# JanWosnitza/FrayTracer

Measured on AMD Instinct MI355X. Metric: Mrays/s (primary+secondary) at 4096x4096; max per-pixel |delta| vs F# ref (delta is measured against the CPU oracle: F# parity is unpinned, DESIGN.md section 2), higher is better.
Workload: dtype f32

## Files before the change

### fraytracer_amd/csrc/ft_kernels.h

```cpp
#pragma once
#include <hip/hip_runtime_api.h>
#include <stddef.h>
#include <stdint.h>

#include "../../include/fraytracer_hip.h"
#include "ft_device.h"
#include "ft_libm.h"

#define FT_BLOCK 256
#define FT_LDS_CNT_WORDS 64
#define FT_LDS_TILE_WORD 40
static_assert(FT_LDS_TILE_WORD >= 36 && FT_LDS_TILE_WORD + 2 * (256 / 64) <= FT_LDS_CNT_WORDS, "the tile words lie behind the clocks, inside the header");
#ifdef FT_UNION_PROFILE
#define FT_LDS_DBG_ROWS 13
#else
#define FT_LDS_DBG_ROWS 0
#endif
#define FT_SH_ROWS 10
#define FT_LDS_SH_BASE (FT_LDS_CNT_WORDS + FT_LDS_DBG_ROWS * FT_BLOCK)
#define FT_LDS_HDR_FLOATS (FT_LDS_SH_BASE + FT_SH_ROWS * FT_BLOCK)
#define FT_CULL_MAX 256
#define FT_CULL_ROW (4 * FT_CULL_MAX)

struct FtLdsLayout { uint32_t slotD, slotL, consts, libmTab, rows, total; };
FT_HD FtLdsLayout ft_lds_layout(uint32_t nSlots, uint32_t nStage, bool libm, bool rows) {
    FtLdsLayout L;
    L.slotD = FT_LDS_HDR_FLOATS;
    L.slotL = FT_LDS_HDR_FLOATS + nSlots * FT_BLOCK;
    L.consts = FT_LDS_HDR_FLOATS + 2u * nSlots * FT_BLOCK;
    L.libmTab = (L.consts + nStage + 1u) & ~1u;
    const uint32_t end = libm ? L.libmTab + 2u * FT_LIBM_TAB_DOUBLES : L.consts + nStage;
    L.rows = (end + 3u) & ~3u;
    L.total = rows ? L.rows + FT_CULL_ROW * (FT_BLOCK / 64) : end;
    return L;
// ... 122 lines not shown
```

### fraytracer_amd/csrc/kernels.hip

```cpp
#include <hip/hip_runtime.h>

#include "../../include/fraytracer_hip.h"
#include "ft_device.h"
#include "ft_kernels.h"
#include "ft_math.h"
#include "ft_libm.h"

#define FT_CONST __attribute__((address_space(4)))
typedef const float FT_CONST* cfp;
template <class T> __device__ __forceinline__ const T FT_CONST* as_const(const T* p) {
    return (const T FT_CONST*)(p);
}

__device__ __forceinline__ f3 ld3(cfp c) { return mk3(c[0], c[1], c[2]); }
__device__ __forceinline__ FtInstr ld_instr(const FtInstr FT_CONST* q) {
    FtInstr r; r.op = q->op; r.dst = q->dst; r.src = q->src; r.type = q->type; r.count = q->count; r.data = q->data;
    r.aux = q->aux; r.flags = q->flags; r.f0 = q->f0; r.f1 = q->f1; r.pad0 = 0; r.pad1 = 0; return r;
}
typedef float v4f __attribute__((ext_vector_type(4)));
typedef uint32_t v4u __attribute__((ext_vector_type(4)));
struct ItemRegs { v4f a; v4u b; };
__device__ __forceinline__ ItemRegs ld_item(const FtItemRec FT_CONST* q) {
    ItemRegs r;
    r.a = *reinterpret_cast<const v4f FT_CONST*>(q);
// ... 345 lines not shown
        uint32_t typeData, mat;
        if (first || (mn > lbA && mn > mdA)) { typeData = ra.b.y; mat = ra.b.z; i += 1u; }
        else {
            if (!(mn > lbA)) break;
            if (j == i || !(mn > lbB)) break;
            i += 2u;
            if (!(mn > mdB)) continue;
            typeData = rb.b.y; mat = rb.b.z;
        }
        FT_UDBG(2, 1); FT_UDBG_WAVE(3);
        FT_UDBG_T0(tPrim);
        float d; uint32_t l;
        ft_candidate<FQ, false>(typeData, mat, consts, p, sd, sl, d, l, [](uint32_t, float&, uint32_t&) {});
        FT_UDBG_T1(9, tPrim);
        if (first) { mn = d; leaf = l; first = false; if (mn <= cap && mn < capBound) break; }
        else {
            if (d < mn) leaf = l;
            mn = ft_min(mn, d);
        }
    }
    FT_UDBG_T1(4, tWalk);
    outD = mn; outLeaf = leaf;
}

#define FT_CULL_NONE 0xffffffffu
#define FT_CULL_NOCLAMP 0x10000u
template <bool WITH_UNION, bool CALLS, int MATH, bool COOP = false>
__device__ __forceinline__ void ft_exec(const FtSceneDev& S, uint32_t pc, uint32_t pcEnd, const f3 p, float* __restrict__ sd,
                                        uint32_t* __restrict__ sl, const float* __restrict__ ldsC, bool fastOk, bool nearOk, float epsHit = __builtin_inff(),
                                        const float* __restrict__ cullRow = nullptr, uint32_t cullN = FT_CULL_NONE);

template <bool FQ, int MATH>
__device__ __forceinline__ void eval_union(const FtSceneDev& S, const FtGrid FT_CONST& g, const f3 p,
                                           float* __restrict__ sd, uint32_t* __restrict__ sl, const float* __restrict__ ldsC,
                                           bool fastOk, bool nearOk, float& outD, uint32_t& outLeaf, float cap, float capBound) {
    const uint32_t cell = g.cellBase + ft_grid_cell(g, p);
    cfp ctr = as_const(S.cellCenters) + 3u * cell;
    const float distanceToCenter = ft_distance(mk3(ctr[0], ctr[1], ctr[2]), p);
    const uint32_t FT_CONST* cellStart = as_const(S.cellStart);
    const FtItemRec FT_CONST* items = as_const(S.items);
    cfp consts = as_const(S.consts);
    uint32_t i = cellStart[cell];
    const uint32_t end = cellStart[cell + 1];

    float mn = 0.0f; uint32_t leaf = 0;
    bool first = true;
// ... 199 lines not shown
__device__ __forceinline__ f3 ft_readlane3(f3 v, int l) {
    return mk3(__int_as_float(__builtin_amdgcn_readlane(__float_as_int(v.x), l)), __int_as_float(__builtin_amdgcn_readlane(__float_as_int(v.y), l)),
               __int_as_float(__builtin_amdgcn_readlane(__float_as_int(v.z), l)));
}
template <int CTRL> __device__ __forceinline__ float ft_dpp(float old, float v) {
    return __int_as_float(__builtin_amdgcn_update_dpp(__float_as_int(old), __float_as_int(v), CTRL, 0xf, 0xf, false));
}
__device__ __forceinline__ float ft_readlane_f(float v, int l) { return __int_as_float(__builtin_amdgcn_readlane(__float_as_int(v), l)); }
__device__ __forceinline__ float ft_wave_max_all(float v) {
    v = __builtin_fmaxf(v, ft_dpp<0x111>(0.0f, v)); v = __builtin_fmaxf(v, ft_dpp<0x112>(0.0f, v));
    v = __builtin_fmaxf(v, ft_dpp<0x114>(0.0f, v)); v = __builtin_fmaxf(v, ft_dpp<0x118>(0.0f, v));
    return __builtin_fmaxf(__builtin_fmaxf(ft_readlane_f(v, 15), ft_readlane_f(v, 31)), __builtin_fmaxf(ft_readlane_f(v, 47), ft_readlane_f(v, 63)));
}
__device__ __forceinline__ float ft_wave_scan_incl(float v, float& total) {
    const uint32_t lane = threadIdx.x & 63u;
    v += ft_dpp<0x111>(0.0f, v); v += ft_dpp<0x112>(0.0f, v); v += ft_dpp<0x114>(0.0f, v); v += ft_dpp<0x118>(0.0f, v);
    const float r0 = ft_readlane_f(v, 15), r1 = ft_readlane_f(v, 31), r2 = ft_readlane_f(v, 47), r3 = ft_readlane_f(v, 63);
    const float p2 = r0 + r1, p3 = p2 + r2;
    v += lane >= 48u ? p3 : (lane >= 32u ? p2 : (lane >= 16u ? r0 : 0.0f));
    total = p3 + r3;
    return v;
}
__device__ __forceinline__ float ft_wave_shift_right1(float v) { return ft_dpp<0x138>(0.0f, v); }
__device__ __forceinline__ uint32_t ft_cull_children(const FtSceneDev& S, const f3 p, bool active, unsigned long long am,
                                                     const float* __restrict__ ldsC, float* __restrict__ row) {
    if (S.cullPc == FT_CULL_NONE) return FT_CULL_NONE;
    const FtInstr FT_CONST* in = as_const(S.instr) + S.cullPc;
    const uint32_t flags = in->flags, count = in->count;
    const float si = in->f0;
    if (in->op != FT_OP_SMOOTH_RUN || !(flags & FT_FLAG_FAST) || count < FT_CULL_MIN || !(si < 0.0f)) return FT_CULL_NONE;
    if (!fast_point_ok(p, active)) return FT_CULL_NONE;
    const uint32_t lane = threadIdx.x & 63u;
    const f3 q00 = ft_readlane3(p, __ffsll((long long)am) - 1);
    const float fx = p.x - q00.x, fy = p.y - q00.y, fz = p.z - q00.z;
    const float far2 = active ? (fx * fx + fy * fy) + fz * fz : 0.0f;
    const float farMax = ft_wave_max_all(far2);
    const unsigned long long fm = __ballot(active && far2 == farMax);
    const f3 q01 = ft_readlane3(p, __ffsll((long long)(fm != 0ull ? fm : am)) - 1);
    const f3 q0 = mk3(0.5f * (q00.x + q01.x), 0.5f * (q00.y + q01.y), 0.5f * (q00.z + q01.z));
    const float ex = p.x - q0.x, ey = p.y - q0.y, ez = p.z - q0.z;
    const float rho2 = ft_wave_max_all(active ? (ex * ex + ey * ey) + ez * ez : 0.0f);
    const float rho = __builtin_amdgcn_sqrtf(rho2) * 1.001f + 1e-6f;
    const uint32_t n = count < FT_CULL_MAX ? count : FT_CULL_MAX;
    const float4* src = reinterpret_cast<const float4*>(ldsC + in->data);
    float4* dst = reinterpret_cast<float4*>(row);
    float carry = 0.0f;
    uint32_t kept = 0;
    bool apart = true;
    for (uint32_t base = 0; base < n; base += 64u) {
// ... 270 lines not shown
    {-0x1.21c850p-1f, 0x1.1e0d66p-3f, -0x1.a00000p-1f}, {0x1.38c4f8p-2f, 0x1.55799ap-3f, -0x1.e00000p-1f}};

struct LaneState {
    uint32_t phase, job, steps, lidx, leaf, outIdx;
    uint32_t certAt;
    f3 o, dir;
    float len, eps;
    uint32_t xs;
    f3 thr;
    uint32_t seed;
    __device__ __forceinline__ uint32_t aoIdx() const { return xs & 255u; }
    __device__ __forceinline__ uint32_t aoOpen() const { return (xs >> 8) & 255u; }
    __device__ __forceinline__ uint32_t bounce() const { return (xs >> 16) & 255u; }
    __device__ __forceinline__ bool inside() const { return (xs >> 31) != 0u; }
};

__device__ __forceinline__ void write_rgb(float* __restrict__ out, uint32_t idx, f3 c) {
    float* o = out + 3ull * idx;
    o[0] = c.x; o[1] = c.y; o[2] = c.z;
}

__device__ __forceinline__ f3 ft_background(const FtRenderArgs& a) { return mk3(a.S.bg[0], a.S.bg[1], a.S.bg[2]); }

template <bool EXT>
__device__ __forceinline__ void emit(const FtRenderArgs& a, const LaneState& s, f3 c) {
    write_rgb(a.out, s.outIdx, EXT ? c * s.thr : c);
}

__device__ __forceinline__ uint32_t ft_glass_hash(uint32_t seed, uint32_t bounce) {
    uint32_t h = seed + (bounce + 1u) * 0x27D4EB2Fu;
    h ^= h >> 16; h *= 0x7FEB352Du; h ^= h >> 15; h *= 0x846CA68Bu; h ^= h >> 16;
    return h;
}

__device__ __forceinline__ void write_try_trace_miss(const FtRenderArgs& a, const LaneState& s) {
    float* o = a.out + 10ull * s.outIdx;
    for (uint32_t i = 0; i < 10u; ++i) o[i] = 0.0f;
}
__device__ __forceinline__ void write_ray(float* o, f3 origin, f3 dir, float len, float eps) {
    o[0] = origin.x; o[1] = origin.y; o[2] = origin.z; o[3] = dir.x; o[4] = dir.y; o[5] = dir.z; o[6] = len; o[7] = eps;
}

template <bool VIEWS = false>
__device__ __forceinline__ bool ends_hit_segment(const FtRenderArgs& a, const LaneState& s) {
    if (VIEWS) return a.hits != 0u && (s.job / a.jobsPerPlane) % a.spp == 0u && s.bounce() == 0u;
    return a.hits != 0u && s.job < a.jobsPerPlane && s.bounce() == 0u;
// ... 221 lines not shown
        holds = holds || (t <= a.occ.reach && nSteps < 131072.0f && hitM <= a.occ.cap && (dist + hitM) * 1.001f < D);
    }
    return ok && holds;
}

__device__ __forceinline__ int first_step_from_cache(LaneState& s) {
    if (s.len <= 0.0f) return 0;
    const float d = *ft_sh(FT_SH_D0);
    if (d != d) { ft_flag(1u); return 2; }
    if (d < s.eps) return 1;
    s.o = s.o + s.dir * d;
    s.len = s.len - d;
    s.steps = 1;
    return 0;
}

struct FtLit { f3 lint, ldir; };
__device__ __forceinline__ FtLit ft_light_at(const uint32_t type, const f3 lv, const f3 lc, const f3 hp) {
    f3 lint = lc, ldir = lv;
    if (type != FT_LIGHT_DIRECTIONAL) { ldir = ft_normalize(lv - hp); lint = lint / ft_length2(lv - hp); }
    return FtLit{lint, ldir};
}

template <bool EXT, int FORM = FT_FORM_FRAME>
__device__ __forceinline__ void settle(const FtRenderArgs& a, LaneState& s) {
    constexpr bool VIEWS = FORM == FT_FORM_VIEWS, SHADE = FORM == FT_FORM_SHADE || FORM == FT_FORM_VIS, VIS = FORM == FT_FORM_VIS;
    const float piInv = 1.0f / 3.14159274101257324f;
    for (;;) {
        if (!SHADE && s.phase == PH_MARCH) {
            if (s.len <= 0.0f || ((!EXT || !s.inside()) && ft_never_enters(a.S, s.o, s.dir, s.eps, s.len))) {
                if (EXT && a.mode == 2u) write_try_trace_miss(a, s);
                else {
                    if (EXT && ends_hit_segment<VIEWS>(a, s)) write_hit_miss(a, hit_index<VIEWS>(a, s));
                    if (!EXT || a.hits != 2u) emit<EXT>(a, s, ft_background(a));
                }
                s.phase = PH_IDLE;
            }
            return;
        }
        if (EXT && s.phase == PH_AO) {
            if (s.len <= 0.0f) { s.xs += 0x101u; s.phase = PH_AONEXT; continue; }
            return;
        }
        if (EXT && s.phase == PH_AONEXT) {
            if (s.aoIdx() >= a.aoSamples) {
                const float f = (float)s.aoOpen() / (float)a.aoSamples;
                sh_set3(FT_SH_LACC, ft_background(a) * f);
                s.lidx = 0; s.phase = PH_LIGHTS;
                continue;
            }
            const f3 dir = ft_normalize(sh_get3(FT_SH_NRM) + mk3(FT_AO_DIRS[s.aoIdx()][0], FT_AO_DIRS[s.aoIdx()][1], FT_AO_DIRS[s.aoIdx()][2]));
            ft_count(FT_C_EXT);
            if (dir.x != dir.x || dir.y != dir.y || dir.z != dir.z) { s.xs += 0x101u; continue; }
            s.o = sh_get3(FT_SH_HP); s.dir = dir; s.len = a.aoRadius; s.steps = 0;
            s.phase = PH_AO;
            if (a.reuse != 0u) {
                const int r = first_step_from_cache(s);
                if (r == 1) { s.xs += 1u; s.phase = PH_AONEXT; }
                else if (r == 2) s.len = -1.0f;
            }
            continue;
        }
        if (s.phase == PH_SHADOW) {
            if (s.len <= 0.0f || ((!EXT || !s.inside()) && ft_never_enters(a.S, s.o, s.dir, s.eps, s.len))) {
                if (VIS) {
                    *ft_vis_word() |= 1u << s.lidx;
                    s.lidx += 1; s.phase = PH_LIGHTS;
                    continue;
                }
                const FtLight L = ld_light(as_const(a.S.lights) + s.lidx);
                const f3 lv = mk3(L.v[0], L.v[1], L.v[2]), hp = sh_get3(FT_SH_HP);
                const FtLit li = ft_light_at(L.type, lv, mk3(L.color[0], L.color[1], L.color[2]), hp);
                sh_set3(FT_SH_LACC, sh_get3(FT_SH_LACC) + li.lint * ft_dot(sh_get3(FT_SH_NRM), li.ldir));
                s.lidx += 1; s.phase = PH_LIGHTS;
                continue;
            }
            return;
        }
        if (s.phase == PH_LIGHTS) {
            if (VIS && s.lidx >= a.S.nLights) {
                a.visOut[s.job] = *ft_vis_word();
                s.phase = PH_IDLE;
                return;
            }
            if (VIS && ((a.visSel >> s.lidx) & 1u) == 0u) { s.lidx += 1; continue; }
            if (!VIS && s.lidx >= a.S.nLights) {
                cfp m = SHADE ? as_const(a.hitsIn) + 16ull * s.job + 11u : as_const(a.S.materials) + 3u * s.leaf;
                const f3 color = mk3(m[0], m[1], m[2]);
                emit<EXT>(a, s, color * (sh_get3(FT_SH_LACC) * piInv));
                s.phase = PH_IDLE;
                return;
            }
            const FtLight L = ld_light(as_const(a.S.lights) + s.lidx);
            const f3 lv = mk3(L.v[0], L.v[1], L.v[2]);
            const f3 hp = sh_get3(FT_SH_HP);
            const f3 ldir = ft_light_at(L.type, lv, mk3(L.color[0], L.color[1], L.color[2]), hp).ldir;
            const float lightCos = ft_dot(sh_get3(FT_SH_NRM), ldir);
            if (lightCos > 0.0f) {
                s.o = hp;
                if (L.type == FT_LIGHT_DIRECTIONAL) {
                    s.dir = lv; s.len = 1000.0f;
                } else {
                    const f3 diff = lv - hp;
                    const float distance2 = ft_length2(diff);
                    s.dir = diff / distance2;
                    s.len = sqrtf(distance2);
                }
                s.steps = 0; ft_count(FT_C_SHADOW);
                s.phase = PH_SHADOW; s.certAt = a.certShadow;
                if (!SHADE && a.reuse != 0u) {
                    const int r = first_step_from_cache(s);
                    if (r == 1) { ft_count(FT_C_HITS); s.lidx += 1; s.phase = PH_LIGHTS; }
                    else if (r == 2) s.len = -1.0f;
                }
                continue;
            }
            s.lidx += 1;
            continue;
        }
        return;
    }
}

struct ViewCam { f3 o, fw, up, rt; float d; uint32_t leaf; };

template <bool EXT, int FORM = FT_FORM_FRAME>
__device__ __forceinline__ void start_job(const FtRenderArgs& a, LaneState& s, const bool camKnown, float dCam, uint32_t leafCam, const ViewCam& vc) {
    constexpr bool VIEWS = FORM == FT_FORM_VIEWS, SHADE = FORM == FT_FORM_SHADE || FORM == FT_FORM_VIS, VIS = FORM == FT_FORM_VIS;
    if (SHADE) {
        const v4f FT_CONST* r = reinterpret_cast<const v4f FT_CONST*>(as_const(a.hitsIn) + 16ull * s.job);
        const v4f r0 = r[0], r1 = r[1], r2 = r[2], r3 = r[3];
        s.outIdx = s.job;
        s.eps = r1.w;
        s.steps = 0;
        const uint32_t kept = VIS ? (a.visIn ? a.visIn[s.job] & a.visKeep : 0u) : 0u;
        if (VIS && __float_as_uint(r3.z) == 0u) {
            a.visOut[s.job] = kept;
            s.phase = PH_IDLE;
            return;
        }
        if (__float_as_uint(r3.z) == 0u) {
            write_rgb(a.out, s.outIdx, ft_background(a));
            s.phase = PH_IDLE;
            return;
        }
        sh_set3(FT_SH_HP, mk3(r0.x, r0.y, r0.z));
        sh_set3(FT_SH_NRM, mk3(r2.x, r2.y, r2.z));
        if (VIS) *ft_vis_word() = kept;
        else sh_set3(FT_SH_LACC, ft_background(a));
        s.lidx = 0;
        s.phase = PH_LIGHTS;
        settle<EXT, FORM>(a, s);
        return;
    }
    if (a.mode >= 1) {
        const ft_ray r = a.rays[s.job];
        s.o = mk3(r.origin.x, r.origin.y, r.origin.z);
        s.dir = mk3(r.direction.x, r.direction.y, r.direction.z);
        s.len = r.length; s.eps = r.epsilon;
        s.outIdx = s.job;
        if (EXT) { s.thr = splat3(1.0f); s.seed = s.job; }
    } else {
        const uint32_t plane = (EXT || VIEWS) ? s.job / a.jobsPerPlane : 0u;
        const uint32_t smp = VIEWS ? (EXT ? plane % a.spp : 0u) : plane, jp = s.job - plane * a.jobsPerPlane;
        const uint32_t t = jp >> 6, i = jp & 63u;
        const uint32_t tx = t / a.tilesY, ty = t - tx * a.tilesY;
        const uint32_t cl = tx * 8u + (i >> 3), y = ty * 8u + (i & 7u);
        if (cl >= (uint32_t)a.nCols || y >= (uint32_t)a.H) { s.phase = PH_IDLE; return; }
        const uint32_t x = (uint32_t)a.x0 + (cl / a.stripeW) * (a.stripeW * a.stripeRanks) + a.stripeRank * a.stripeW + cl % a.stripeW;
        const float ox = EXT ? (float)(smp % a.sppN) / (float)a.sppN : 0.0f, oy = EXT ? (float)(smp / a.sppN) / (float)a.sppN : 0.0f;
        const float px = EXT ? ((float)x + ox) / a.maxSize : (float)x / a.maxSize;
        const float py = EXT ? ((float)y + oy) / a.maxSize : (float)y / a.maxSize;
        const f3 fw = VIEWS ? vc.fw : mk3(a.cam[3], a.cam[4], a.cam[5]), up = VIEWS ? vc.up : mk3(a.cam[6], a.cam[7], a.cam[8]);
        const f3 rt = VIEWS ? vc.rt : mk3(a.cam[9], a.cam[10], a.cam[11]);
        s.o = VIEWS ? vc.o : mk3(a.cam[0], a.cam[1], a.cam[2]);
        s.dir = ft_normalize(fw + (px - 0.5f) * rt + (py - 0.5f) * up);
        s.len = a.length; s.eps = a.eps;
        s.outIdx = plane * a.planePixels + cl * (uint32_t)a.H + y;
        if (VIEWS) { dCam = vc.d; leafCam = vc.leaf; }
        if (EXT) {
            s.thr = splat3(1.0f);
            if (a.spectral != 0u) { const uint32_t bin = smp % a.spectral; s.thr = mk3(a.spec[bin][0], a.spec[bin][1], a.spec[bin][2]); }
            s.seed = x * 0x9E3779B1u + y * 0x85EBCA77u + smp * 0xC2B2AE3Du;
        }
    }
    if (EXT) s.xs &= 0xffffu;
    s.steps = 0; ft_count(FT_C_PRIMARY);
    s.phase = PH_MARCH; s.certAt = a.certPrim;
    if (camKnown && s.len > 0.0f) {
        if (dCam != dCam) { ft_flag(1u); s.len = -1.0f; }
        else if (dCam < s.eps) { ft_count(FT_C_HITP); s.leaf = leafCam; s.phase = PH_NX; }
        else { s.o = s.o + s.dir * dCam; s.len = s.len - dCam; s.steps = 1; }
    }
    settle<EXT, FORM>(a, s);
}

__device__ __forceinline__ void glass_bounce(const FtRenderArgs& a, LaneState& s) {
    cfp mx = as_const(a.materialsExt) + 4u * s.leaf;
    const bool glass = mx[0] != 0.0f;
    const f3 black = mk3(0.0f, 0.0f, 0.0f);
    if (!glass) {
        if (s.inside()) { write_rgb(a.out, s.outIdx, black); s.phase = PH_IDLE; }
        return;
    }
    const f3 N = sh_get3(FT_SH_NRM), D = s.dir, hp = sh_get3(FT_SH_HP);
    if (s.bounce() >= a.maxBounces || N.x != N.x || N.y != N.y || N.z != N.z) { write_rgb(a.out, s.outIdx, black); s.phase = PH_IDLE; return; }
    float cosi = -ft_dot(N, D);
    if (!(cosi > 0.0f)) cosi = 0.0f;
    float n = mx[1];
    if (a.spectral != 0u) {
        const uint32_t smp = s.job / a.jobsPerPlane;
        n = mx[1] + mx[2] * a.spec[smp % a.spectral][3];
    }
    const float n1 = !s.inside() ? 1.0f : n, n2 = !s.inside() ? n : 1.0f;
    const float eta = n1 / n2;
    const float k = 1.0f - (eta * eta) * (1.0f - cosi * cosi);
    bool reflect = true;
// ... 2 lines not shown
        cost = sqrtf(k);
        float rs, rp;
        { const float p = n2 * cosi, q = n1 * cost, x = (p - q) / (p + q); rs = x * x; }
        { const float p = n1 * cosi, q = n2 * cost, x = (p - q) / (p + q); rp = x * x; }
        const float reflectance = 0.5f * (rs + rp);
        const float u = (float)(ft_glass_hash(s.seed, s.bounce()) >> 8) * (1.0f / 16777216.0f);
        reflect = u < reflectance;
    }
    ft_count(FT_C_EXT);
    if (reflect) {
        s.dir = ft_normalize(D + N * (2.0f * cosi));
        s.o = hp + N * (2.0f * s.eps);
    } else {
        s.dir = ft_normalize(D * eta + N * (eta * cosi - cost));
        s.o = hp - N * (4.0f * s.eps);
        s.xs ^= 0x80000000u;
        if (s.inside()) { cfp t = as_const(a.S.materials) + 3u * s.leaf; s.thr = s.thr * mk3(t[0], t[1], t[2]); }
    }
    s.xs += 0x10000u;
    s.len = a.length; s.steps = 0;
    s.phase = PH_MARCH; s.certAt = a.certPrim;
}

__device__ __forceinline__ unsigned long long wave_sum(uint32_t v) {
    unsigned long long x = v;
    for (int off = 32; off > 0; off >>= 1) x += __shfl_down(x, off, 64);
    return x;
}

template <int VARIANT, bool EXT, int MATH = 0, int K = 0, int FORM = FT_FORM_FRAME>
__device__ __forceinline__ void ft_trace_body(const FtRenderArgs& a) {
    constexpr bool VIEWS = FORM == FT_FORM_VIEWS, SHADE = FORM == FT_FORM_SHADE || FORM == FT_FORM_VIS;
    static_assert(!SHADE || !EXT, "ft_shade_hits and ft_light_visibility have no EXTENSION build");
    const uint32_t tid = threadIdx.x, lane = tid & 63u;
    unsigned long long* clk0 = reinterpret_cast<unsigned long long*>(ft_lds + 32);
    if (blockIdx.x == 0 && tid == 0) { clk0[0] = clock64(); clk0[1] = wall_clock64(); }
    const FtLdsLayout L = ft_lds_layout(a.S.nSlots, a.S.nStage, MATH != 0, true);
    float* sd = ft_lds + L.slotD + tid;
    uint32_t* sl = reinterpret_cast<uint32_t*>(ft_lds + L.slotL) + tid;
    float* ldsC = ft_lds + L.consts;
    for (uint32_t i = tid; i < a.S.nStage; i += FT_BLOCK) ldsC[i] = a.S.consts[i];
    if (MATH != 0 && tid < FT_LIBM_TAB_DOUBLES) const_cast<ft_u64*>(ft_libm_tab(a.S))[tid] = ft_libm_tab_g[tid];
    if (tid < 32u) reinterpret_cast<uint32_t*>(ft_lds)[tid] = 0u;
#ifdef FT_UNION_PROFILE
    for (uint32_t k = 0; k < FT_LDS_DBG_ROWS; ++k) reinterpret_cast<uint32_t*>(ft_lds)[FT_LDS_CNT_WORDS + tid + k * FT_BLOCK] = 0u;
#endif
    __syncthreads();

    float* coopRow = ft_lds + ft_lds_layout(a.S.nSlots, a.S.nStage, MATH != 0, true).rows + (uint32_t)__builtin_amdgcn_readfirstlane((int)(tid >> 6)) * FT_CULL_ROW;
    uint32_t cullSkipped = 0, cullTotal = 0;
    uint32_t chunkNext = 0, chunkEnd = 0;
    uint32_t waveEvals = 0;
    constexpr bool ORDER = FORM == FT_FORM_FRAME && !EXT && VARIANT == 1;
    uint32_t* tileSt = reinterpret_cast<uint32_t*>(ft_lds) + FT_LDS_TILE_WORD + (tid >> 6);
    constexpr uint32_t TILE_EVALS = FT_BLOCK / 64;
    if (ORDER && lane == 0) tileSt[0] = 0xffffffffu;
    uint32_t coopEvals = 0;
    uint32_t nEvals = 0;
    bool exhausted = false;
    LaneState s;
    s.phase = PH_IDLE; s.job = 0; s.steps = 0; s.lidx = 0; s.leaf = 0; s.outIdx = 0; s.certAt = 0xffffffffu;
    s.o = s.dir = mk3(0, 0, 0);
    s.len = 0; s.eps = 0;
    s.xs = 0;
    s.thr = splat3(1.0f); s.seed = 0;
    bool camKnown = false;
    float dCam = 0.0f; uint32_t leafCam = 0u;
    if (!SHADE && a.reuse != 0u && a.mode == 0u) {
        s.phase = PH_CAM;
        if (VIEWS) { const float* c = a.views + 12u * (lane % a.nViews); s.o = mk3(c[0], c[1], c[2]); }
        else s.o = mk3(a.cam[0], a.cam[1], a.cam[2]);
        s.eps = a.eps;
    }
    ViewCam vc{};

    for (;;) {
        for (int round = 0; round < 3; ++round) {
            const unsigned long long idle = __ballot(s.phase == PH_IDLE);
            if (idle == 0ull) break;
            if ((uint32_t)__popcll(idle) < a.refillMin && __ballot(s.phase >= PH_MARCH) != 0ull) break;
            if (chunkNext == chunkEnd) {
                if (exhausted) break;
                if (ORDER && a.tileCost != nullptr && lane == 0) {
                    const uint32_t t = tileSt[0];
                    if (t < (a.nJobs >> 6)) a.tileCost[t] = waveEvals - tileSt[TILE_EVALS];
                    tileSt[0] = 0xffffffffu;
                }
                uint32_t base = 0, take = a.chunk;
                if (lane == 0) {
                    if (a.shrink1 < a.nJobs) {
                        const uint32_t cur = __hip_atomic_load(a.counter, __ATOMIC_RELAXED, __HIP_MEMORY_SCOPE_AGENT);
                        take = cur >= a.shrink2 ? a.chunk / 4u : (cur >= a.shrink1 ? a.chunk / 2u : a.chunk);
                    }
                    base = atomicAdd(a.counter, take);
                }
                base = __builtin_amdgcn_readfirstlane(base);
                const uint32_t took = (uint32_t)__builtin_amdgcn_readfirstlane((int)take);
                if (base >= a.nJobs) { exhausted = true; break; }
                chunkNext = base;
                chunkEnd = (a.nJobs - base < took) ? a.nJobs : base + took;
                if (ORDER && a.tileCost != nullptr) {
                    uint32_t tile = base >> 6;
                    if (a.tileOrder != nullptr) {
                        tile = (uint32_t)__builtin_amdgcn_readfirstlane((int)a.tileOrder[tile]);
                        chunkNext = tile << 6; chunkEnd = chunkNext + 64u;
                    }
                    if (lane == 0) { tileSt[0] = tile; tileSt[TILE_EVALS] = waveEvals; }
                }
            }
            uint32_t avail = chunkEnd - chunkNext;
            if (VIEWS && a.mode == 0u) {
                const uint32_t jobsPerView = a.jobsPerPlane * (EXT ? a.spp : 1u);
                const uint32_t v = chunkNext / jobsPerView, viewEnd = (v + 1u) * jobsPerView;
                if (viewEnd - chunkNext < avail) avail = viewEnd - chunkNext;
                cfp c = as_const(a.views) + 12u * v;
                vc.o = ld3(c); vc.fw = ld3(c + 3); vc.up = ld3(c + 6); vc.rt = ld3(c + 9);
                vc.d = ft_readlane_f(dCam, (int)v); vc.leaf = (uint32_t)__builtin_amdgcn_readlane((int)leafCam, (int)v);
            }
            const uint32_t nIdle = (uint32_t)__popcll(idle);
            const uint32_t rank = (uint32_t)__popcll(idle & ((1ull << lane) - 1ull));
            if (s.phase == PH_IDLE && rank < avail) { s.job = chunkNext + rank; start_job<EXT, FORM>(a, s, camKnown, dCam, leafCam, vc); }
            chunkNext += (nIdle < avail) ? nIdle : avail;
        }
        if (s.phase == PH_IDLE && exhausted && chunkNext == chunkEnd) s.phase = PH_DONE;
        if (__ballot(s.phase != PH_DONE) == 0ull) break;

        if (VARIANT == 1 && a.occPeriod != 0u && waveEvals % a.occPeriod == 0u) {
            const bool cand = s.phase == PH_SHADOW && s.steps - a.occFrom < a.occPeriod && (!EXT || !s.inside());
            if ((uint32_t)__popcll(__ballot(cand)) >= a.occMin) {
                const bool hit = ft_occlusion_certificate(a, ldsC + 0, cand, s.o, s.dir, s.eps, s.len, s.steps);
                if (hit) { ft_count(FT_C_HITS); s.lidx += 1; s.phase = PH_LIGHTS; settle<EXT, FORM>(a, s); }
                if (__ballot(hit) != 0ull && __ballot(s.phase >= PH_MARCH) == 0ull) continue;
            }
        }

        if (VARIANT == 1 && a.cert != 0u) {
            bool ends = false;
            if (a.bundlePeriod != 0u && waveEvals % a.bundlePeriod == 0u) {
#pragma unroll 1
                for (uint32_t ph = SHADE ? PH_SHADOW : PH_MARCH; ph <= PH_SHADOW; ph += PH_SHADOW - PH_MARCH) {
                    const bool cand = s.phase == ph && (ph == PH_MARCH || s.steps >= a.bundleShadow) && (!EXT || !s.inside());
                    if ((uint32_t)__popcll(__ballot(cand)) < a.bundleMin) continue;
                    if (ft_bundle_certificate(a.S, ldsC + 0, cand, s.o, s.dir, s.eps, s.len, s.steps, a.bundleMin)) ends = true;
                }
            }
            const bool due = !ends && (s.phase == PH_MARCH || s.phase == PH_SHADOW) && s.steps >= s.certAt && (!EXT || !s.inside());
            bool tried = false;
            if ((uint32_t)__popcll(__ballot(due)) >= a.certMin) {
                tried = true;
                const bool holds = ft_miss_certificate(a.S, ldsC + 0, due, s.o, s.dir, s.eps, s.len, s.steps);
                if (due) {
                    if (holds) ends = true;
                    else s.certAt = a.certRepeat != 0u ? s.steps + a.certRepeat : 0xffffffffu;
                }
            }
            if (ends) { s.len = -1.0f; settle<EXT, FORM>(a, s); }
            if ((tried || __ballot(ends) != 0ull) && __ballot(s.phase >= PH_MARCH) == 0ull) continue;
        }

        const bool active = s.phase >= PH_MARCH;
        waveEvals += 1;
        FT_UDBG_T0(tRound);
        auto query_point = [&]() {
            f3 q = s.o;
            if (!SHADE && s.phase >= PH_NX && s.phase <= PH_NC) {
                const f3 base = s.o + s.dir * (-s.eps);
                const float h = s.eps * 0.125f;
                q = base;
                if (s.phase == PH_NX) q.x = base.x + h;
                if (s.phase == PH_NY) q.y = base.y + h;
                if (s.phase == PH_NZ) q.z = base.z + h;
            }
            return q;
        };
        const unsigned long long am = __ballot(active);
        const bool camRound = __ballot(s.phase == PH_CAM) != 0ull;
        if (!camRound) nEvals += (uint32_t)__popcll(am);
        const bool coop = (uint32_t)__popcll(am) <= a.tailK;
        float dCoop = 0.0f; uint32_t leafCoop = 0;
        if (coop && am != 0ull) {
            const f3 qm = query_point();
            if (VARIANT == 1) {
                ft_eval_smooth_spheres_packed<MATH>(a.S, qm, active, am, (uint32_t)__popcll(am), ldsC, coopRow, dCoop, leafCoop);
                if (!camRound) coopEvals += (uint32_t)__popcll(am);
            } else {
                unsigned long long m = am;
                while (m != 0ull) {
                    const int L = __ffsll((long long)m) - 1;
                    m &= m - 1ull;
                    const f3 qL = ft_readlane3(qm, L);
                    float dL; uint32_t leafL;
                    if (VARIANT == 3) ft_eval_carved<K, true>(a.S, a.carve, qL, dL, leafL, __builtin_inff());
                    else ft_eval<VARIANT == 2, MATH, true>(a.S, qL, sd, sl, ldsC, dL, leafL);
                    if ((int)lane == L) { dCoop = dL; leafCoop = leafL; }
                    if (!camRound) coopEvals += 1;
                }
            }
        }
        uint32_t cullN = FT_CULL_NONE;
        if (VARIANT != 3 && a.cull != 0u && !coop && am != 0ull) {
            cullN = ft_cull_children(a.S, query_point(), active, am, ldsC, coopRow);
            if (cullN != FT_CULL_NONE) {
                const uint32_t cnt = (as_const(a.S.instr) + a.S.cullPc)->count;
                const uint32_t looked = cnt < FT_CULL_MAX ? cnt : FT_CULL_MAX;
                cullTotal += looked * (uint32_t)__popcll(am) >> 6; cullSkipped += (looked - (cullN & 0xffffu)) * (uint32_t)__popcll(am) >> 6;
            }
        }
        if (active) {
            float d; uint32_t leaf;
            FT_UDBG_T0(tEval);
            if (coop) { d = dCoop; leaf = leafCoop; }
            else {
                const f3 q = query_point();
                if (VARIANT == 1) ft_eval_smooth_spheres<MATH>(a.S, q, ldsC, d, leaf, coopRow, cullN);
                else if (VARIANT == 3) ft_eval_carved<K>(a.S, a.carve, q, d, leaf, a.lazy == 0u ? __builtin_inff() : s.eps);
                else ft_eval<VARIANT == 2, MATH>(a.S, q, sd, sl, ldsC, d, leaf,
                                                  (EXT && s.inside()) || a.lazy == 0u ? __builtin_inff() : s.eps, coopRow, cullN);
            }
            FT_UDBG_T1(5, tEval); FT_UDBG_WAVE(6);
            if (EXT) d = __uint_as_float(__float_as_uint(d) ^ (s.xs & 0x80000000u));

            const uint32_t ph = SHADE ? (uint32_t)PH_SHADOW : s.phase;
            switch (ph) {
            case PH_MARCH:
            case PH_SHADOW:
            case PH_AO: {
                bool miss = false;
                if (d != d) { ft_flag(1u); miss = true; }
// ... 29 lines not shown
            case PH_NZ: *ft_sh(FT_SH_NRM + 2) = d; s.phase = PH_NC; break;
            case PH_NC: {
                *ft_sh(FT_SH_D0) = d;
                const f3 nrm = ft_normalize(sh_get3(FT_SH_NRM) - splat3(d));
                const f3 hp = s.o + s.dir * (-s.eps);
                sh_set3(FT_SH_NRM, nrm);
                sh_set3(FT_SH_HP, hp);
                sh_set3(FT_SH_LACC, ft_background(a));
                s.lidx = 0;
                s.phase = PH_LIGHTS;
                if (EXT && ends_hit_segment<VIEWS>(a, s)) {
                    cfp m = as_const(a.S.materials) + 3u * s.leaf;
                    const float len = s.len - (-s.eps);
                    write_hit_record(a, hit_index<VIEWS>(a, s), v4f{hp.x, hp.y, hp.z, s.dir.x}, v4f{s.dir.y, s.dir.z, len, s.eps},
                                     v4f{nrm.x, nrm.y, nrm.z, m[0]}, v4f{m[1], m[2], __int_as_float(1), 0.0f}, as_const(a.matHandles)[s.leaf]);
                    if (a.hits == 2u) s.phase = PH_IDLE;
                }
                if (EXT && a.aoSamples != 0u) { s.xs &= 0xffff0000u; s.phase = PH_AONEXT; }
                if (EXT && a.maxBounces != 0u) glass_bounce(a, s);
                break;
            }
            default: break;
            }
            settle<EXT, FORM>(a, s);
        }
        FT_UDBG_T1(7, tRound);
    }

    const uint32_t* cw = reinterpret_cast<const uint32_t*>(ft_lds) + (tid >> 6);
    const unsigned long long e = nEvals, sh = cw[FT_C_SHADOW * 4], hp = cw[FT_C_HITP * 4], hs = cw[FT_C_HITS * 4], pr = cw[FT_C_PRIMARY * 4], ex = cw[FT_C_EXT * 4];
    const unsigned long long fl = cw[FT_C_FLAGS * 4] & 3u, fc = cw[FT_C_FLAGS * 4] & 4u;
    if (lane == 0) {
        atomicAdd(&a.stats->sdf_evals, e);
        atomicAdd(&a.stats->rays_shadow, sh);
        atomicAdd(&a.stats->hits_primary, hp);
        atomicAdd(&a.stats->hits_shadow, hs);
        atomicAdd(&a.stats->rays_primary, pr);
        if (ex) atomicAdd(&a.stats->rays_ext, ex);
        atomicAdd(&a.stats->wave_evals, (unsigned long long)waveEvals);
        if (coopEvals) atomicAdd(&a.stats->coop_evals, (unsigned long long)coopEvals);
        if (cullTotal) { atomicAdd(&a.stats->cull_total, (unsigned long long)cullTotal); atomicAdd(&a.stats->cull_skipped, (unsigned long long)cullSkipped); }
        if (fl | fc) atomicOr(&a.stats->flags, fl | fc);
        if (blockIdx.x == 0 && tid == 0) { atomicAdd(&a.stats->clk_shader, clock64() - clk0[0]); atomicAdd(&a.stats->clk_ref, wall_clock64() - clk0[1]); }
    }
#ifdef FT_UNION_PROFILE
    for (uint32_t k = 0; k < 12; ++k) {
        const unsigned long long v = wave_sum(reinterpret_cast<const uint32_t*>(ft_lds)[FT_LDS_CNT_WORDS + tid + k * FT_BLOCK]);
        if (lane == 0 && v) atomicAdd(&ft_union_dbg[k], v);
    }
#endif
}

#ifndef FT_GENERAL_WAVES
#define FT_GENERAL_WAVES 6
#endif
#define FT_OCC(n) __attribute__((amdgpu_waves_per_eu(n, n)))
#ifndef FT_CALLS_WAVES
#define FT_CALLS_WAVES 5
#endif
#ifndef FT_EXT_WAVES
#define FT_EXT_WAVES 5
#endif
#define FT_CALLS_OCC FT_OCC(FT_CALLS_WAVES)
#define FT_EXT_OCC FT_OCC(FT_EXT_WAVES)

#define FT_TRACE_BUILDS(X, ...) \
// ... 701 lines not shown
```

Measured before the change: 1136.

## Cut SGPR pressure in lean smooth-sphere trace by re-reading kernargs and LDS counters

For the VARIANT==1, non-EXT build this adds a LEAN mode. Rarely used kernel arguments are reloaded from the kernarg segment at their point of use, behind opaque asm barriers, so the compiler does not keep them live in scalar registers across the main loop. Per-wave statistics counters (evals, coop evals, cull totals) move from registers into LDS words updated by lane-0 atomics, and the block-0 clock report becomes an LDS flag. The aim is to lower register pressure and spilling, or to raise occupancy, in exchange for extra scalar loads and LDS atomics on every round.

```diff
diff --git a/fraytracer_amd/csrc/ft_kernels.h b/fraytracer_amd/csrc/ft_kernels.h
--- a/fraytracer_amd/csrc/ft_kernels.h
+++ b/fraytracer_amd/csrc/ft_kernels.h
@@ -10,6 +10,9 @@
 #define FT_BLOCK 256
 #define FT_LDS_CNT_WORDS 64
 #define FT_LDS_TILE_WORD 40
+#define FT_LDS_WAVE_WORD 48
+#define FT_LDS_REPORT_WORD 36
+static_assert(FT_LDS_WAVE_WORD >= FT_LDS_TILE_WORD + 2 * (256 / 64) && FT_LDS_WAVE_WORD + 4 * (256 / 64) <= FT_LDS_CNT_WORDS, "the wave sums lie behind the tile words, inside the header");
 static_assert(FT_LDS_TILE_WORD >= 36 && FT_LDS_TILE_WORD + 2 * (256 / 64) <= FT_LDS_CNT_WORDS, "the tile words lie behind the clocks, inside the header");
 #ifdef FT_UNION_PROFILE
 #define FT_LDS_DBG_ROWS 13
diff --git a/fraytracer_amd/csrc/kernels.hip b/fraytracer_amd/csrc/kernels.hip
--- a/fraytracer_amd/csrc/kernels.hip
+++ b/fraytracer_amd/csrc/kernels.hip
@@ -391,6 +391,12 @@
     FT_UDBG_T1(4, tWalk);
     outD = mn; outLeaf = leaf;
 }
+
+__device__ __forceinline__ uint32_t ft_word_held(uint32_t v) {
+    asm volatile("" : "+s"(v));
+    return v;
+}
+#define FT_WORD_AT_USE(on, v) ((on) ? ft_word_held(v) : (v))
 
 #define FT_CULL_NONE 0xffffffffu
 #define FT_CULL_NOCLAMP 0x10000u
@@ -636,9 +642,10 @@
     return v;
 }
 __device__ __forceinline__ float ft_wave_shift_right1(float v) { return ft_dpp<0x138>(0.0f, v); }
+template <bool HELD = false>
 __device__ __forceinline__ uint32_t ft_cull_children(const FtSceneDev& S, const f3 p, bool active, unsigned long long am,
                                                      const float* __restrict__ ldsC, float* __restrict__ row) {
-    if (S.cullPc == FT_CULL_NONE) return FT_CULL_NONE;
+    if (FT_WORD_AT_USE(HELD, S.cullPc) == FT_CULL_NONE) return FT_CULL_NONE;
     const FtInstr FT_CONST* in = as_const(S.instr) + S.cullPc;
     const uint32_t flags = in->flags, count = in->count;
     const float si = in->f0;
@@ -955,6 +962,13 @@
 
 __device__ __forceinline__ f3 ft_background(const FtRenderArgs& a) { return mk3(a.S.bg[0], a.S.bg[1], a.S.bg[2]); }
 
+__device__ __forceinline__ const FtRenderArgs& ft_args_reread() {
+    const FtRenderArgs FT_CONST* p = (const FtRenderArgs FT_CONST*)__builtin_amdgcn_kernarg_segment_ptr();
+    asm volatile("" : "+s"(p));
+    return *(const FtRenderArgs*)p;
+}
+#define FT_ARGS_AT_USE(on, a) ((on) ? ft_args_reread() : (a))
+
 template <bool EXT>
 __device__ __forceinline__ void emit(const FtRenderArgs& a, const LaneState& s, f3 c) {
     write_rgb(a.out, s.outIdx, EXT ? c * s.thr : c);
@@ -1222,17 +1236,19 @@
     return FtLit{lint, ldir};
 }
 
-template <bool EXT, int FORM = FT_FORM_FRAME>
+template <bool EXT, int FORM = FT_FORM_FRAME, bool LEAN = false>
 __device__ __forceinline__ void settle(const FtRenderArgs& a, LaneState& s) {
     constexpr bool VIEWS = FORM == FT_FORM_VIEWS, SHADE = FORM == FT_FORM_SHADE || FORM == FT_FORM_VIS, VIS = FORM == FT_FORM_VIS;
     const float piInv = 1.0f / 3.14159274101257324f;
+    const FtRenderArgs* u = &a;
     for (;;) {
         if (!SHADE && s.phase == PH_MARCH) {
             if (s.len <= 0.0f || ((!EXT || !s.inside()) && ft_never_enters(a.S, s.o, s.dir, s.eps, s.len))) {
-                if (EXT && a.mode == 2u) write_try_trace_miss(a, s);
+                if (LEAN) u = &ft_args_reread();
+                if (EXT && u->mode == 2u) write_try_trace_miss(*u, s);
                 else {
-                    if (EXT && ends_hit_segment<VIEWS>(a, s)) write_hit_miss(a, hit_index<VIEWS>(a, s));
-                    if (!EXT || a.hits != 2u) emit<EXT>(a, s, ft_background(a));
+                    if (EXT && ends_hit_segment<VIEWS>(*u, s)) write_hit_miss(*u, hit_index<VIEWS>(*u, s));
+                    if (!EXT || u->hits != 2u) emit<EXT>(*u, s, ft_background(*u));
                 }
                 s.phase = PH_IDLE;
             }
@@ -1263,12 +1279,13 @@
         }
         if (s.phase == PH_SHADOW) {
             if (s.len <= 0.0f || ((!EXT || !s.inside()) && ft_never_enters(a.S, s.o, s.dir, s.eps, s.len))) {
+                if (LEAN) u = &ft_args_reread();
                 if (VIS) {
                     *ft_vis_word() |= 1u << s.lidx;
                     s.lidx += 1; s.phase = PH_LIGHTS;
                     continue;
                 }
-                const FtLight L = ld_light(as_const(a.S.lights) + s.lidx);
+                const FtLight L = ld_light(as_const(u->S.lights) + s.lidx);
                 const f3 lv = mk3(L.v[0], L.v[1], L.v[2]), hp = sh_get3(FT_SH_HP);
                 const FtLit li = ft_light_at(L.type, lv, mk3(L.color[0], L.color[1], L.color[2]), hp);
                 sh_set3(FT_SH_LACC, sh_get3(FT_SH_LACC) + li.lint * ft_dot(sh_get3(FT_SH_NRM), li.ldir));
@@ -1278,20 +1295,21 @@
             return;
         }
         if (s.phase == PH_LIGHTS) {
-            if (VIS && s.lidx >= a.S.nLights) {
-                a.visOut[s.job] = *ft_vis_word();
+            if (LEAN) u = &ft_args_reread();
+            if (VIS && s.lidx >= u->S.nLights) {
+                u->visOut[s.job] = *ft_vis_word();
                 s.phase = PH_IDLE;
                 return;
             }
-            if (VIS && ((a.visSel >> s.lidx) & 1u) == 0u) { s.lidx += 1; continue; }
-            if (!VIS && s.lidx >= a.S.nLights) {
-                cfp m = SHADE ? as_const(a.hitsIn) + 16ull * s.job + 11u : as_const(a.S.materials) + 3u * s.leaf;
+            if (VIS && ((u->visSel >> s.lidx) & 1u) == 0u) { s.lidx += 1; continue; }
+            if (!VIS && s.lidx >= u->S.nLights) {
+                cfp m = SHADE ? as_const(u->hitsIn) + 16ull * s.job + 11u : as_const(u->S.materials) + 3u * s.leaf;
                 const f3 color = mk3(m[0], m[1], m[2]);
-                emit<EXT>(a, s, color * (sh_get3(FT_SH_LACC) * piInv));
+                emit<EXT>(*u, s, color * (sh_get3(FT_SH_LACC) * piInv));
                 s.phase = PH_IDLE;
                 return;
             }
-            const FtLight L = ld_light(as_const(a.S.lights) + s.lidx);
+            const FtLight L = ld_light(as_const(u->S.lights) + s.lidx);
             const f3 lv = mk3(L.v[0], L.v[1], L.v[2]);
             const f3 hp = sh_get3(FT_SH_HP);
             const f3 ldir = ft_light_at(L.type, lv, mk3(L.color[0], L.color[1], L.color[2]), hp).ldir;
@@ -1307,8 +1325,8 @@
                     s.len = sqrtf(distance2);
                 }
                 s.steps = 0; ft_count(FT_C_SHADOW);
-                s.phase = PH_SHADOW; s.certAt = a.certShadow;
-                if (!SHADE && a.reuse != 0u) {
+                s.phase = PH_SHADOW; s.certAt = u->certShadow;
+                if (!SHADE && u->reuse != 0u) {
                     const int r = first_step_from_cache(s);
                     if (r == 1) { ft_count(FT_C_HITS); s.lidx += 1; s.phase = PH_LIGHTS; }
                     else if (r == 2) s.len = -1.0f;
@@ -1324,9 +1342,10 @@
 
 struct ViewCam { f3 o, fw, up, rt; float d; uint32_t leaf; };
 
-template <bool EXT, int FORM = FT_FORM_FRAME>
-__device__ __forceinline__ void start_job(const FtRenderArgs& a, LaneState& s, const bool camKnown, float dCam, uint32_t leafCam, const ViewCam& vc) {
+template <bool EXT, int FORM = FT_FORM_FRAME, bool LEAN = false>
+__device__ __forceinline__ void start_job(const FtRenderArgs& a_, LaneState& s, const bool camKnown, float dCam, uint32_t leafCam, const ViewCam& vc) {
     constexpr bool VIEWS = FORM == FT_FORM_VIEWS, SHADE = FORM == FT_FORM_SHADE || FORM == FT_FORM_VIS, VIS = FORM == FT_FORM_VIS;
+    const FtRenderArgs& a = FT_ARGS_AT_USE(LEAN, a_);
     if (SHADE) {
         const v4f FT_CONST* r = reinterpret_cast<const v4f FT_CONST*>(as_const(a.hitsIn) + 16ull * s.job);
         const v4f r0 = r[0], r1 = r[1], r2 = r[2], r3 = r[3];
@@ -1350,7 +1369,7 @@
         else sh_set3(FT_SH_LACC, ft_background(a));
         s.lidx = 0;
         s.phase = PH_LIGHTS;
-        settle<EXT, FORM>(a, s);
+        settle<EXT, FORM, LEAN>(a_, s);
         return;
     }
     if (a.mode >= 1) {
@@ -1392,7 +1411,7 @@
         else if (dCam < s.eps) { ft_count(FT_C_HITP); s.leaf = leafCam; s.phase = PH_NX; }
         else { s.o = s.o + s.dir * dCam; s.len = s.len - dCam; s.steps = 1; }
     }
-    settle<EXT, FORM>(a, s);
+    settle<EXT, FORM, LEAN>(a_, s);
 }
 
 __device__ __forceinline__ void glass_bounce(const FtRenderArgs& a, LaneState& s) {
@@ -1441,6 +1460,10 @@
     s.phase = PH_MARCH; s.certAt = a.certPrim;
 }
 
+__device__ __forceinline__ void ft_wave_word_add(uint32_t* word, uint32_t v) {
+    if ((threadIdx.x & 63u) == 0u) __hip_atomic_fetch_add(word, v, __ATOMIC_RELAXED, __HIP_MEMORY_SCOPE_WORKGROUP);
+}
+
 __device__ __forceinline__ unsigned long long wave_sum(uint32_t v) {
     unsigned long long x = v;
     for (int off = 32; off > 0; off >>= 1) x += __shfl_down(x, off, 64);
@@ -1451,6 +1474,7 @@
 __device__ __forceinline__ void ft_trace_body(const FtRenderArgs& a) {
     constexpr bool VIEWS = FORM == FT_FORM_VIEWS, SHADE = FORM == FT_FORM_SHADE || FORM == FT_FORM_VIS;
     static_assert(!SHADE || !EXT, "ft_shade_hits and ft_light_visibility have no EXTENSION build");
+    constexpr bool LEAN = VARIANT == 1 && !EXT;
     const uint32_t tid = threadIdx.x, lane = tid & 63u;
     unsigned long long* clk0 = reinterpret_cast<unsigned long long*>(ft_lds + 32);
     if (blockIdx.x == 0 && tid == 0) { clk0[0] = clock64(); clk0[1] = wall_clock64(); }
@@ -1460,11 +1484,12 @@
     float* ldsC = ft_lds + L.consts;
     for (uint32_t i = tid; i < a.S.nStage; i += FT_BLOCK) ldsC[i] = a.S.consts[i];
     if (MATH != 0 && tid < FT_LIBM_TAB_DOUBLES) const_cast<ft_u64*>(ft_libm_tab(a.S))[tid] = ft_libm_tab_g[tid];
-    if (tid < 32u) reinterpret_cast<uint32_t*>(ft_lds)[tid] = 0u;
+    if (tid < 32u || (LEAN && (tid - FT_LDS_WAVE_WORD < 4u * (FT_BLOCK / 64) || tid == FT_LDS_REPORT_WORD))) reinterpret_cast<uint32_t*>(ft_lds)[tid] = 0u;
 #ifdef FT_UNION_PROFILE
     for (uint32_t k = 0; k < FT_LDS_DBG_ROWS; ++k) reinterpret_cast<uint32_t*>(ft_lds)[FT_LDS_CNT_WORDS + tid + k * FT_BLOCK] = 0u;
 #endif
     __syncthreads();
+    if (LEAN && blockIdx.x == 0 && tid == 0) reinterpret_cast<uint32_t*>(ft_lds)[FT_LDS_REPORT_WORD] = 1u;
 
     float* coopRow = ft_lds + ft_lds_layout(a.S.nSlots, a.S.nStage, MATH != 0, true).rows + (uint32_t)__builtin_amdgcn_readfirstlane((int)(tid >> 6)) * FT_CULL_ROW;
     uint32_t cullSkipped = 0, cullTotal = 0;
@@ -1476,6 +1501,8 @@
     if (ORDER && lane == 0) tileSt[0] = 0xffffffffu;
     uint32_t coopEvals = 0;
     uint32_t nEvals = 0;
+    uint32_t* waveSt = reinterpret_cast<uint32_t*>(ft_lds) + FT_LDS_WAVE_WORD + (tid >> 6);
+    enum : uint32_t { ST_EVALS = 0, ST_COOP = FT_BLOCK / 64, ST_CULL_TOTAL = 2 * (FT_BLOCK / 64), ST_CULL_SKIPPED = 3 * (FT_BLOCK / 64) };
     bool exhausted = false;
     LaneState s;
     s.phase = PH_IDLE; s.job = 0; s.steps = 0; s.lidx = 0; s.leaf = 0; s.outIdx = 0; s.certAt = 0xffffffffu;
@@ -1500,28 +1527,29 @@
             if ((uint32_t)__popcll(idle) < a.refillMin && __ballot(s.phase >= PH_MARCH) != 0ull) break;
             if (chunkNext == chunkEnd) {
                 if (exhausted) break;
-                if (ORDER && a.tileCost != nullptr && lane == 0) {
+                const FtRenderArgs& u = FT_ARGS_AT_USE(LEAN, a);
+                if (ORDER && u.tileCost != nullptr && lane == 0) {
                     const uint32_t t = tileSt[0];
-                    if (t < (a.nJobs >> 6)) a.tileCost[t] = waveEvals - tileSt[TILE_EVALS];
+                    if (t < (u.nJobs >> 6)) u.tileCost[t] = waveEvals - tileSt[TILE_EVALS];
                     tileSt[0] = 0xffffffffu;
                 }
-                uint32_t base = 0, take = a.chunk;
+                uint32_t base = 0, take = u.chunk;
                 if (lane == 0) {
-                    if (a.shrink1 < a.nJobs) {
-                        const uint32_t cur = __hip_atomic_load(a.counter, __ATOMIC_RELAXED, __HIP_MEMORY_SCOPE_AGENT);
-                        take = cur >= a.shrink2 ? a.chunk / 4u : (cur >= a.shrink1 ? a.chunk / 2u : a.chunk);
+                    if (u.shrink1 < u.nJobs) {
+                        const uint32_t cur = __hip_atomic_load(u.counter, __ATOMIC_RELAXED, __HIP_MEMORY_SCOPE_AGENT);
+                        take = cur >= u.shrink2 ? u.chunk / 4u : (cur >= u.shrink1 ? u.chunk / 2u : u.chunk);
                     }
-                    base = atomicAdd(a.counter, take);
+                    base = atomicAdd(u.counter, take);
                 }
                 base = __builtin_amdgcn_readfirstlane(base);
                 const uint32_t took = (uint32_t)__builtin_amdgcn_readfirstlane((int)take);
-                if (base >= a.nJobs) { exhausted = true; break; }
+                if (base >= u.nJobs) { exhausted = true; break; }
                 chunkNext = base;
-                chunkEnd = (a.nJobs - base < took) ? a.nJobs : base + took;
-                if (ORDER && a.tileCost != nullptr) {
+                chunkEnd = (u.nJobs - base < took) ? u.nJobs : base + took;
+                if (ORDER && u.tileCost != nullptr) {
                     uint32_t tile = base >> 6;
-                    if (a.tileOrder != nullptr) {
-                        tile = (uint32_t)__builtin_amdgcn_readfirstlane((int)a.tileOrder[tile]);
+                    if (u.tileOrder != nullptr) {
+                        tile = (uint32_t)__builtin_amdgcn_readfirstlane((int)u.tileOrder[tile]);
                         chunkNext = tile << 6; chunkEnd = chunkNext + 64u;
                     }
                     if (lane == 0) { tileSt[0] = tile; tileSt[TILE_EVALS] = waveEvals; }
@@ -1538,42 +1566,43 @@
             }
             const uint32_t nIdle = (uint32_t)__popcll(idle);
             const uint32_t rank = (uint32_t)__popcll(idle & ((1ull << lane) - 1ull));
-            if (s.phase == PH_IDLE && rank < avail) { s.job = chunkNext + rank; start_job<EXT, FORM>(a, s, camKnown, dCam, leafCam, vc); }
+            if (s.phase == PH_IDLE && rank < avail) { s.job = chunkNext + rank; start_job<EXT, FORM, LEAN>(a, s, camKnown, dCam, leafCam, vc); }
             chunkNext += (nIdle < avail) ? nIdle : avail;
         }
         if (s.phase == PH_IDLE && exhausted && chunkNext == chunkEnd) s.phase = PH_DONE;
         if (__ballot(s.phase != PH_DONE) == 0ull) break;
 
-        if (VARIANT == 1 && a.occPeriod != 0u && waveEvals % a.occPeriod == 0u) {
+        if (VARIANT == 1 && FT_WORD_AT_USE(LEAN, a.occPeriod) != 0u && waveEvals % a.occPeriod == 0u) {
             const bool cand = s.phase == PH_SHADOW && s.steps - a.occFrom < a.occPeriod && (!EXT || !s.inside());
             if ((uint32_t)__popcll(__ballot(cand)) >= a.occMin) {
-                const bool hit = ft_occlusion_certificate(a, ldsC + 0, cand, s.o, s.dir, s.eps, s.len, s.steps);
-                if (hit) { ft_count(FT_C_HITS); s.lidx += 1; s.phase = PH_LIGHTS; settle<EXT, FORM>(a, s); }
+                const bool hit = ft_occlusion_certificate(FT_ARGS_AT_USE(LEAN, a), ldsC + 0, cand, s.o, s.dir, s.eps, s.len, s.steps);
+                if (hit) { ft_count(FT_C_HITS); s.lidx += 1; s.phase = PH_LIGHTS; settle<EXT, FORM, LEAN>(a, s); }
                 if (__ballot(hit) != 0ull && __ballot(s.phase >= PH_MARCH) == 0ull) continue;
             }
         }
 
-        if (VARIANT == 1 && a.cert != 0u) {
+        if (VARIANT == 1 && FT_WORD_AT_USE(LEAN, a.cert) != 0u) {
             bool ends = false;
-            if (a.bundlePeriod != 0u && waveEvals % a.bundlePeriod == 0u) {
+            if (FT_WORD_AT_USE(LEAN, a.bundlePeriod) != 0u && waveEvals % a.bundlePeriod == 0u) {
 #pragma unroll 1
                 for (uint32_t ph = SHADE ? PH_SHADOW : PH_MARCH; ph <= PH_SHADOW; ph += PH_SHADOW - PH_MARCH) {
                     const bool cand = s.phase == ph && (ph == PH_MARCH || s.steps >= a.bundleShadow) && (!EXT || !s.inside());
                     if ((uint32_t)__popcll(__ballot(cand)) < a.bundleMin) continue;
-                    if (ft_bundle_certificate(a.S, ldsC + 0, cand, s.o, s.dir, s.eps, s.len, s.steps, a.bundleMin)) ends = true;
+                    if (ft_bundle_certificate(FT_ARGS_AT_USE(LEAN, a).S, ldsC + 0, cand, s.o, s.dir, s.eps, s.len, s.steps, a.bundleMin)) ends = true;
                 }
             }
             const bool due = !ends && (s.phase == PH_MARCH || s.phase == PH_SHADOW) && s.steps >= s.certAt && (!EXT || !s.inside());
             bool tried = false;
             if ((uint32_t)__popcll(__ballot(due)) >= a.certMin) {
                 tried = true;
-                const bool holds = ft_miss_certificate(a.S, ldsC + 0, due, s.o, s.dir, s.eps, s.len, s.steps);
+                const FtRenderArgs& u = FT_ARGS_AT_USE(LEAN, a);
+                const bool holds = ft_miss_certificate(u.S, ldsC + 0, due, s.o, s.dir, s.eps, s.len, s.steps);
                 if (due) {
                     if (holds) ends = true;
-                    else s.certAt = a.certRepeat != 0u ? s.steps + a.certRepeat : 0xffffffffu;
+                    else s.certAt = u.certRepeat != 0u ? s.steps + u.certRepeat : 0xffffffffu;
                 }
             }
-            if (ends) { s.len = -1.0f; settle<EXT, FORM>(a, s); }
+            if (ends) { s.len = -1.0f; settle<EXT, FORM, LEAN>(a, s); }
             if ((tried || __ballot(ends) != 0ull) && __ballot(s.phase >= PH_MARCH) == 0ull) continue;
         }
 
@@ -1594,14 +1623,16 @@
         };
         const unsigned long long am = __ballot(active);
         const bool camRound = __ballot(s.phase == PH_CAM) != 0ull;
-        if (!camRound) nEvals += (uint32_t)__popcll(am);
+        if (LEAN) { if (!camRound) ft_wave_word_add(waveSt + ST_EVALS, (uint32_t)__popcll(am)); }
+        else if (!camRound) nEvals += (uint32_t)__popcll(am);
         const bool coop = (uint32_t)__popcll(am) <= a.tailK;
         float dCoop = 0.0f; uint32_t leafCoop = 0;
         if (coop && am != 0ull) {
             const f3 qm = query_point();
             if (VARIANT == 1) {
                 ft_eval_smooth_spheres_packed<MATH>(a.S, qm, active, am, (uint32_t)__popcll(am), ldsC, coopRow, dCoop, leafCoop);
-                if (!camRound) coopEvals += (uint32_t)__popcll(am);
+                if (LEAN) { if (!camRound) ft_wave_word_add(waveSt + ST_COOP, (uint32_t)__popcll(am)); }
+                else if (!camRound) coopEvals += (uint32_t)__popcll(am);
             } else {
                 unsigned long long m = am;
                 while (m != 0ull) {
@@ -1617,12 +1648,14 @@
             }
         }
         uint32_t cullN = FT_CULL_NONE;
-        if (VARIANT != 3 && a.cull != 0u && !coop && am != 0ull) {
-            cullN = ft_cull_children(a.S, query_point(), active, am, ldsC, coopRow);
+        if (VARIANT != 3 && FT_WORD_AT_USE(LEAN, a.cull) != 0u && !coop && am != 0ull) {
+            cullN = ft_cull_children<LEAN>(a.S, query_point(), active, am, ldsC, coopRow);
             if (cullN != FT_CULL_NONE) {
                 const uint32_t cnt = (as_const(a.S.instr) + a.S.cullPc)->count;
                 const uint32_t looked = cnt < FT_CULL_MAX ? cnt : FT_CULL_MAX;
-                cullTotal += looked * (uint32_t)__popcll(am) >> 6; cullSkipped += (looked - (cullN & 0xffffu)) * (uint32_t)__popcll(am) >> 6;
+                const uint32_t total = looked * (uint32_t)__popcll(am) >> 6, skipped = (looked - (cullN & 0xffffu)) * (uint32_t)__popcll(am) >> 6;
+                if (LEAN) { ft_wave_word_add(waveSt + ST_CULL_TOTAL, total); ft_wave_word_add(waveSt + ST_CULL_SKIPPED, skipped); }
+                else { cullTotal += total; cullSkipped += skipped; }
             }
         }
         if (active) {
@@ -1698,26 +1731,28 @@
             }
             default: break;
             }
-            settle<EXT, FORM>(a, s);
+            settle<EXT, FORM, LEAN>(a, s);
         }
         FT_UDBG_T1(7, tRound);
     }
 
     const uint32_t* cw = reinterpret_cast<const uint32_t*>(ft_lds) + (tid >> 6);
+    if (LEAN) { nEvals = waveSt[ST_EVALS]; coopEvals = waveSt[ST_COOP]; cullTotal = waveSt[ST_CULL_TOTAL]; cullSkipped = waveSt[ST_CULL_SKIPPED]; }
     const unsigned long long e = nEvals, sh = cw[FT_C_SHADOW * 4], hp = cw[FT_C_HITP * 4], hs = cw[FT_C_HITS * 4], pr = cw[FT_C_PRIMARY * 4], ex = cw[FT_C_EXT * 4];
     const unsigned long long fl = cw[FT_C_FLAGS * 4] & 3u, fc = cw[FT_C_FLAGS * 4] & 4u;
     if (lane == 0) {
-        atomicAdd(&a.stats->sdf_evals, e);
-        atomicAdd(&a.stats->rays_shadow, sh);
-        atomicAdd(&a.stats->hits_primary, hp);
-        atomicAdd(&a.stats->hits_shadow, hs);
-        atomicAdd(&a.stats->rays_primary, pr);
-        if (ex) atomicAdd(&a.stats->rays_ext, ex);
-        atomicAdd(&a.stats->wave_evals, (unsigned long long)waveEvals);
-        if (coopEvals) atomicAdd(&a.stats->coop_evals, (unsigned long long)coopEvals);
-        if (cullTotal) { atomicAdd(&a.stats->cull_total, (unsigned long long)cullTotal); atomicAdd(&a.stats->cull_skipped, (unsigned long long)cullSkipped); }
-        if (fl | fc) atomicOr(&a.stats->flags, fl | fc);
-        if (blockIdx.x == 0 && tid == 0) { atomicAdd(&a.stats->clk_shader, clock64() - clk0[0]); atomicAdd(&a.stats->clk_ref, wall_clock64() - clk0[1]); }
+        const FtRenderArgs& u = FT_ARGS_AT_USE(LEAN, a);
+        atomicAdd(&u.stats->sdf_evals, e);
+        atomicAdd(&u.stats->rays_shadow, sh);
+        atomicAdd(&u.stats->hits_primary, hp);
+        atomicAdd(&u.stats->hits_shadow, hs);
+        atomicAdd(&u.stats->rays_primary, pr);
+        if (ex) atomicAdd(&u.stats->rays_ext, ex);
+        atomicAdd(&u.stats->wave_evals, (unsigned long long)waveEvals);
+        if (coopEvals) atomicAdd(&u.stats->coop_evals, (unsigned long long)coopEvals);
+        if (cullTotal) { atomicAdd(&u.stats->cull_total, (unsigned long long)cullTotal); atomicAdd(&u.stats->cull_skipped, (unsigned long long)cullSkipped); }
+        if (fl | fc) atomicOr(&u.stats->flags, fl | fc);
+        if (LEAN ? (tid == 0 && reinterpret_cast<const uint32_t*>(ft_lds)[FT_LDS_REPORT_WORD] != 0u) : (blockIdx.x == 0 && tid == 0)) { atomicAdd(&u.stats->clk_shader, clock64() - clk0[0]); atomicAdd(&u.stats->clk_ref, wall_clock64() - clk0[1]); }
     }
 #ifdef FT_UNION_PROFILE
     for (uint32_t k = 0; k < 12; ++k) {
```

New measurement: 1209, median of 6. 1.06x the previous value.
